# peterWon/D-LIOM

Measured on AMD Instinct MI355X. Metric: scans/sec (64-beam x 1024 pts -> 10 cm 3D submap), higher is better.
Workload: dtype f32 transforms + u16 voxels/u64 sums (rtcsm), f64 (ceres); 1 GPU; config2 W-dense: 64x1024 scan, all returns matched (adaptive voxel filters neutralised), RTCSM3D + CeresScanMatcher3D(hi+lo) + insertion(hi+lo); N_hi=65536, N_lo=65536, C=35937, linear_window=1, angular_window=5, rescored_candidates_last=2, box_kernel_variant=0, map_scans=20, grids_inserted_into=2, parallelism=replicas x1

## Files before the change

d-liom_amd/csrc/internal.h:

```cpp
#ifndef DLIOM_CSRC_INTERNAL_H_
#define DLIOM_CSRC_INTERNAL_H_

#include <hip/hip_runtime.h>

#include <chrono>
#include <cstddef>
#include <cstdint>
#include <memory>
#include <string>
#include <vector>

#include "../../include/dliom.h"
#include "pinned_layout.h"

namespace dliom {

void set_last_error(const char* what, hipError_t e, const char* file, int line);

#define DLIOM_HIP_TRY(expr)                                          \
  do {                                                               \
    hipError_t _e = (expr);                                          \
    if (_e != hipSuccess) {                                          \
      ::dliom::set_last_error(#expr, _e, __FILE__, __LINE__);        \
      return DLIOM_ERR_HIP;                                          \
// ... 89 lines not shown
  int64_t read_backs = 0;
  int64_t poll_fallbacks = 0;
  int64_t host_syncs = 0;
  dliom::DevBuf batch;
  dliom::DevBuf icp_batch;
  dliom::DevBuf ndt_batch;
  dliom::DevBuf ndt_target_batch;
  dliom::DevBuf nn_index_batch;
  dliom::DevBuf xray_leaves, xray_cells;
  dliom::DevBuf surf, surf_out;
  dliom::DevBuf painter;
  int64_t painter_launches = 0, painter_pairs = 0, painter_texels_uploaded = 0;
  dliom::DevBuf compress, compress_out;
  bool surf_tables_ready = false;
  dliom::DevBuf outlier;
  void* batch_pinned = nullptr;
  size_t batch_pinned_bytes = 0;
  int reserve_batch_pinned(size_t bytes);
  int num_cus = 256;
  unsigned func_attr_set = 0;
  hipStream_t aux_stream = nullptr;
  hipEvent_t aux_fork = nullptr;
  dliom::DevBuf aux_scratch;
  void* aux_pinned = nullptr;
  int aux_histogram_size = 0;
  unsigned aux_seq = 0;
  bool aux_enqueued = false;
  const dliom_cloud* aux_cloud = nullptr;
  float aux_rotation[4] = {1.f, 0.f, 0.f, 0.f};
  bool aux_has_rotation = false;
  bool hist_expect_big = true;
  int hist_poll_us = 150;
  std::chrono::steady_clock::time_point hist_enqueued_at;
  hipStream_t hist_big_stream = nullptr;
  hipEvent_t hist_fork = nullptr, hist_join = nullptr;
  bool profiling = false;
  unsigned profiling_mask = ~0u;
  struct Span {
    hipEvent_t a, b;
    int id;
  };
  std::vector<Span> spans;
  std::vector<hipEvent_t> event_pool;
  double kernel_ms[DLIOM_KERNEL_COUNT] = {};
  int64_t kernel_launches[DLIOM_KERNEL_COUNT] = {};
  dliom_rtcsm_stats last_rtcsm = {};
  void* rtcsm_state = nullptr;
  void (*rtcsm_state_free)(void*) = nullptr;

  int begin_span(int id);
  void end_span(int span);
  int collect_spans();
};

struct dliom_grid {
  dliom_ctx* ctx = nullptr;
  float resolution = 0.f;
  int bits = 1;
  uint32_t* d_table = nullptr;
  uint16_t* d_pool = nullptr;
  int32_t* d_slot_coord = nullptr;
  uint32_t* d_count = nullptr;
  int64_t capacity = 0;
  int64_t used_upper = 1;
  unsigned* h_count_slot = nullptr;
  unsigned insert_seq = 0, applied_seq = 0;
// ... 127 lines not shown
int device_block_alloc(int device, size_t need, void** p, size_t* bytes);
void device_block_free(int device, void* p, size_t bytes);
struct CompactScratch {
  unsigned *keep, *inclusive, *max_sq;
  int* index;
  void* tmp;
  size_t tmp_bytes;
  void* extra;
};
int carve_compact(dliom_ctx* ctx, int64_t n, CompactScratch* s, size_t extra_bytes = 0, size_t zeroed_extra_bytes = 0);
int empty_cloud(dliom_ctx* ctx, dliom_cloud** out);
int max_of_kept(dliom_ctx* ctx, const float* x, const float* y, const float* z, int64_t n, const CompactScratch& s);
int scan_kept(dliom_ctx* ctx, int64_t n, const CompactScratch& s);
int read_kept(dliom_ctx* ctx, int64_t n, const CompactScratch& s, const GatherJob* more, int64_t* kept, float* max_sq,
              unsigned* more_host);
int emit_kept(dliom_ctx* ctx, const float* x, const float* y, const float* z, int64_t n, const CompactScratch& s, int64_t kept,
              float max_sq, dliom_cloud** out, int32_t* kept_index);
int compact_kept(dliom_ctx* ctx, const dliom_cloud* in, const CompactScratch& s, const unsigned* flag_word, unsigned* flag,
                 dliom_cloud** out, int32_t* kept_index, int64_t capacity, int64_t* num_kept);
int gather_batch_attributes(dliom_ctx* ctx, const int* d_index, int64_t kept, const float* src_intensities, const float* src_colors,
                            float* dst_intensities, float* dst_colors);
int compact_batch(dliom_points_batch* batch, const CompactScratch& s, const unsigned* flag_word, unsigned* flag, int64_t* num_kept);
struct DevicePoints {
  const float4* xyzt;
  const float* intensities;
};
int assemble_from_sensor_points(dliom_ctx* ctx, dliom_trajectory* traj, int64_t cloud_time, const float* points_xyzt, const DevicePoints* device_points,
                                int64_t n, const double sensor_to_tracking[7], dliom_cloud** out, float origin[3], int32_t* kept_index,
                                int64_t capacity, int64_t* num_kept, const float* intensities, AttrBlock* kept_intensities);
int timed_cloud_view(const dliom_timed_cloud* cloud, const dliom_ctx* ctx, int64_t* n, const float4** d_xyzt, const float** d_intensities,
                     float* front_t);
int timed_cloud_origin_index(const dliom_timed_cloud* cloud, bool* has, const float** d_origin_index);
int std_sort_order_enqueue(dliom_ctx* ctx, const float* d_keys, int n, const int** d_order, const int** d_status);
int launch_sequential_sums(dliom_ctx* ctx, int method, const GridView& gv, const dliom_cloud& cloud, const float4* d_rot,
                           int R, const float* d_trans, const unsigned* d_list, const unsigned* d_count, unsigned count,
                           DevBuf* scratch, float* d_ksums);
int sequential_sum_method(int64_t num_points);
int sequential_probability_sums(dliom_ctx* ctx, const dliom_cloud& cloud, const dliom_grid* grid, const float* poses7,
                                int k, float* sums);
struct SequentialSumJob {
  const dliom_cloud* cloud;
  const dliom_grid* grid;
  int first, k;
};
int sequential_probability_sums_enqueue(dliom_ctx* ctx, const SequentialSumJob* jobs, int num_jobs, const float4* d_rot,
                                        const float* d_trans, const unsigned* d_list, float* d_sums);
}

#endif
```

d-liom_amd/csrc/rtcsm3d.hip:

```cpp
#include <algorithm>
#include <cmath>
#include <cstdio>
#include <cstdlib>
#include <cstring>
#include <type_traits>
#include <vector>

#include <dlfcn.h>
#include <rccl/rccl.h>

#include "device_common.h"
#include "host_math.h"
#include "probability_values.h"
#include "rtcsm_candidates.h"
#include "score_box.h"

namespace dliom {

constexpr int kBlock = 256;

template <int PPT, bool WIDE = false>
__global__ __launch_bounds__(kBlock) void rtcsm_score_kernel(
    GridView g, const float* __restrict__ px, const float* __restrict__ py,
    const float* __restrict__ pz, const float4* __restrict__ rot, int R, int r_first, int r_last,
    const float* __restrict__ trans, int T, int rots_per_block,
    unsigned long long* __restrict__ sums) {
  extern __shared__ unsigned block_sum[];
  float x[PPT], y[PPT], z[PPT];
#pragma unroll
  for (int k = 0; k < PPT; ++k) {
    const int i = (blockIdx.x * PPT + k) * kBlock + threadIdx.x;
    x[k] = px[i];
    y[k] = py[i];
    z[k] = pz[i];
  }
  const int r_begin = r_first + blockIdx.y * rots_per_block;
  const int r_end = min(r_begin + rots_per_block, r_last);
  const int lane = threadIdx.x & 63;
  const float inv = g.inv_resolution;
  typedef typename std::conditional<WIDE, unsigned long long, unsigned>::type idx_t;
  const idx_t sentinel = static_cast<idx_t>(1) << (3 * g.log2_leaves);
  const unsigned lb = static_cast<unsigned>(g.log2_leaves);
  for (int r = r_begin; r < r_end; ++r) {
    for (int j = threadIdx.x; j < T; j += kBlock) block_sum[j] = 0u;
    __syncthreads();
    const float4 qq = rot[r];
// ... 215 lines not shown
              ox[k] = lds_off[min(max(cell_of(rx[k] + t.x, g.resolution) + to_table, 0), TS - 1)];
              oy[k] = lds_off[TS + min(max(cell_of(ry[k] + t.y, g.resolution) + to_table, 0), TS - 1)];
              oz[k] = lds_off[2 * TS + min(max(cell_of(rz[k] + t.z, g.resolution) + to_table, 0), TS - 1)];
            }
          }
        }
        unsigned v[P];
#pragma unroll
        for (int k = 0; k < P; ++k)
          v[k] = *reinterpret_cast<const unsigned short*>(reinterpret_cast<const char*>(g.dense) + (ox[k] + oy[k] + oz[k]));
        unsigned a = 0;
#pragma unroll
        for (int k = 0; k < P; ++k) a += v[k];
        atomicAdd(&lds_acc[jj * bs + threadIdx.x], a);
      }
    }
    if (active) {
      for (int jj = 0; jj < tc; ++jj)
        atomicAdd(&sums[static_cast<size_t>(jc + jj) * R + r],
                  static_cast<unsigned long long>(lds_acc[jj * bs + threadIdx.x]));
    }
  }
}

struct BoundParams {
  double a;
  double b;
  double delta;
  double wt, wr;
  int n;
  int n_pad;
  int R, T;
  int r_first, r_last;
};

__device__ double seq_sum_error_bound(int n, double U) {
  double err = 0.0;
  long long i = 0;
  for (int k = -4; k < 64 && i < n; ++k) {
    const double top = ldexp(1.0, k + 1);
    long long last;
    if (U < top) {
      last = n;
    } else {
      last = static_cast<long long>(floor(top / 0.93)) - 1;
      if (last > n) last = n;
    }
    if (last > i) {
      err += 0.5 * ldexp(1.0, k - 23) * static_cast<double>(last - i);
      i = last;
    }
  }
  return err;
}

__device__ __forceinline__ float next_up(float f) { return __uint_as_float(__float_as_uint(f) + 1u); }
__device__ __forceinline__ float next_down(float f) {
  const unsigned u = __float_as_uint(f);
  return u == 0u ? 0.f : __uint_as_float(u - 1u);
}

__global__ void rtcsm_bounds_kernel(const unsigned long long* __restrict__ sums, long long C,
                                    const float* __restrict__ t_norm, const float* __restrict__ r_angle,
                                    BoundParams p, float* __restrict__ lo, float* __restrict__ hi,
                                    unsigned* __restrict__ best_lo_bits) {
  const long long c = static_cast<long long>(blockIdx.x) * blockDim.x + threadIdx.x;
  const bool in_range = c < C;
  const int j = in_range ? static_cast<int>(c / p.R) : 0, r = in_range ? static_cast<int>(c % p.R) : 0;
  const bool mine = in_range && r >= p.r_first && r < p.r_last;
  float flo = 0.f, fhi = -1.f;
  if (mine) {
  const double s = static_cast<double>(sums[c] - static_cast<unsigned long long>(p.n_pad));
  const double mid = p.a * s + p.b * p.n;
  const double slack = p.delta * p.n + 1e-9 * mid;
  double sum_lo = mid - slack, sum_hi = mid + slack;
  const double U = sum_hi * (1.0 + 1.0 / 32.0);
  const double e = seq_sum_error_bound(p.n, U);
  if (sum_hi + e > U || p.n > (1 << 19)) {
    flo = 0.f;
    fhi = 3.0e38f;
  } else {
    sum_lo -= e;
    sum_hi += e;
    const double arg = static_cast<double>(t_norm[j]) * p.wt + static_cast<double>(r_angle[r]) * p.wr;
    const double pen = exp(-(arg * arg));
    const float nf = static_cast<float>(p.n);
    float qlo = next_down(next_down(static_cast<float>(sum_lo))) / nf;
    float qhi = next_up(next_up(static_cast<float>(sum_hi))) / nf;
    qlo = next_down(qlo);
    qhi = next_up(qhi);
    flo = next_down(next_down(static_cast<float>(static_cast<double>(qlo) * pen * (1.0 - 1e-9))));
    fhi = next_up(next_up(static_cast<float>(static_cast<double>(qhi) * pen * (1.0 + 1e-9))));
    if (!(flo > 0.f)) flo = 0.f;
  }
  }
  if (in_range) {
    lo[c] = flo;
    hi[c] = fhi;
  }
  unsigned best = __float_as_uint(flo);
#pragma unroll
  for (int off = 32; off > 0; off >>= 1) best = max(best, static_cast<unsigned>(__shfl_xor(static_cast<int>(best), off, 64)));
  if ((threadIdx.x & 63) == 0 && best != 0u) atomicMax(best_lo_bits, best);
}

__global__ void rtcsm_select_kernel(const float* __restrict__ hi, long long C,
                                    const unsigned* __restrict__ best_lo_bits,
                                    unsigned* __restrict__ count, unsigned* __restrict__ list) {
  const long long c = static_cast<long long>(blockIdx.x) * blockDim.x + threadIdx.x;
  if (c >= C) return;
// ... 640 lines not shown
                       const dliom_cloud& cloud, const dliom_grid* grid, int shard, int num_shards,
                       unsigned* local_best_lo_bits) {
#ifdef DLIOM_EXPERIMENTS
  g_host_prep.start();
#endif
  if (cloud.n <= 0) return DLIOM_ERR_EMPTY_CLOUD;
  if (cloud.n > (1 << 27) || num_shards < 1 || shard < 0 || shard >= num_shards)
    return DLIOM_ERR_INVALID_ARGUMENT;
  RtcsmState* st = state_of(ctx);
  st->active = false;
  st->o = *o;
  st->cloud = cloud;
  st->grid = grid;
  std::memcpy(st->init7, init7, sizeof st->init7);
  st->shard = shard;
  st->num_shards = num_shards;
  st->used_box = false;
  Candidates& c = st->c;
  generate_candidates(*o, grid->resolution, cloud.max_norm, init7, &c);
  DLIOM_PREP_LAP(0);
  const int64_t C = c.w.num_candidates;
  const int R = static_cast<int>(c.w.num_rotations), T = static_cast<int>(c.w.num_translations);
  if (C <= 0 || C > (int64_t{1} << 31)) return DLIOM_ERR_INVALID_ARGUMENT;
  st->r_first = static_cast<int>(static_cast<int64_t>(R) * shard / num_shards);
  st->r_last = static_cast<int>(static_cast<int64_t>(R) * (shard + 1) / num_shards);

  const size_t bytes_f = align256(static_cast<size_t>(C) * 4);
  DLIOM_TRY(ctx->bounds.reserve(3 * bytes_f + 256));
  char* bb = static_cast<char*>(ctx->bounds.p);
  float* d_lo = reinterpret_cast<float*>(bb);
  st->d_hi = reinterpret_cast<float*>(bb + bytes_f);
  st->d_list = reinterpret_cast<unsigned*>(bb + 2 * bytes_f);
  st->d_ctrs = reinterpret_cast<unsigned*>(bb + 3 * bytes_f);
  const FillJob zero_ctrs{st->d_ctrs, 8, 0u};
  if (st->r_last <= st->r_first) DLIOM_TRY(fill_multi(ctx, &zero_ctrs, 1));
  if (st->r_last > st->r_first) {
    int64_t pad_processed = 0;
    DLIOM_TRY(run_score_volume(ctx, cloud, grid, c, st->r_first, st->r_last, &st->d, &st->d_sums,
                               &pad_processed, &zero_ctrs));
    st->used_box = ctx->last_score_used_box;
    const LutModel& lm = lut_model();
    BoundParams bp;
    bp.a = lm.a;
    bp.b = lm.b;
    bp.delta = lm.delta;
    bp.wt = o->translation_delta_cost_weight;
    bp.wr = o->rotation_delta_cost_weight;
    bp.n = static_cast<int>(cloud.n);
    bp.n_pad = static_cast<int>(pad_processed);
    bp.R = R;
    bp.T = T;
    bp.r_first = st->r_first;
    bp.r_last = st->r_last;
    const unsigned cblocks = static_cast<unsigned>((C + 255) / 256);
    const int span = ctx->begin_span(DLIOM_KERNEL_RTCSM_SELECT);
    hipLaunchKernelGGL(rtcsm_bounds_kernel, dim3(cblocks), dim3(256), 0, ctx->stream, st->d_sums,
                       static_cast<long long>(C), st->d.t_norm, st->d.r_angle, bp, d_lo, st->d_hi,
                       st->d_ctrs);
    ctx->end_span(span);
    DLIOM_HIP_TRY(hipGetLastError());
  }
  if (local_best_lo_bits != nullptr) {
    unsigned* h_err = pinned_at<unsigned>(ctx, kPinBoxErrorWord);
    *h_err = 0u;
    DLIOM_HIP_TRY(hipMemcpyAsync(local_best_lo_bits, st->d_ctrs, 4, hipMemcpyDeviceToHost, ctx->stream));
    if (st->used_box)
      DLIOM_HIP_TRY(hipMemcpyAsync(h_err, static_cast<char*>(ctx->box_error.p) + 4, 4, hipMemcpyDeviceToHost, ctx->stream));
    DLIOM_HIP_TRY(hipStreamSynchronize(ctx->stream));
    bool overflow = false;
    DLIOM_TRY(box_overflowed(ctx, *h_err, &overflow));
    if (overflow && !ctx->force_dense_score) {
      ctx->force_dense_score = true;
      const dliom_rtcsm_options o_copy = st->o;
      const int s = match_begin(ctx, &o_copy, init7, cloud, grid, shard, num_shards, local_best_lo_bits);
      ctx->force_dense_score = false;
      return s;
    }
  }
  st->active = true;
  return DLIOM_OK;
}

static int match_finish(dliom_ctx* ctx, const unsigned* global_best_lo_bits, uint64_t* local_best_packed) {
  RtcsmState* st = state_of(ctx);
  if (!st->active) return DLIOM_ERR_INVALID_ARGUMENT;
  const dliom_rtcsm_options* o = &st->o;
  const Candidates& c = st->c;
  const int64_t C = c.w.num_candidates;
  const int R = static_cast<int>(c.w.num_rotations);
  const dliom_cloud& cloud = st->cloud;
  st->best_score = -1.f;
  st->best_c = -1;
  unsigned K = 0;
  if (st->r_last > st->r_first) {
    if (global_best_lo_bits != nullptr) {
      DLIOM_HIP_TRY(hipMemcpyAsync(st->d_ctrs, global_best_lo_bits, 4, hipMemcpyHostToDevice, ctx->stream));
    }
    const unsigned cblocks = static_cast<unsigned>((C + 255) / 256);
    int span = ctx->begin_span(DLIOM_KERNEL_RTCSM_SELECT);
    hipLaunchKernelGGL(rtcsm_select_kernel, dim3(cblocks), dim3(256), 0, ctx->stream, st->d_hi,
                       static_cast<long long>(C), st->d_ctrs, st->d_ctrs + 1, st->d_list);
    ctx->end_span(span);
    DLIOM_HIP_TRY(hipGetLastError());
  }
  constexpr unsigned kSpecK = 8;
  std::vector<unsigned> list;
  std::vector<float> ksums;
  if (st->r_last > st->r_first) {
    static_assert((2 + 2 * kSpecK + 1) * 4 <= kPinMatchReadback.bytes, "the read-back fits its region");
    unsigned* h_ctrs = pinned_at<unsigned>(ctx, kPinMatchReadback);
    unsigned* h_list = h_ctrs + 2;
    float* h_sums = reinterpret_cast<float*>(h_ctrs + 2 + kSpecK);
    auto rescore = [&](unsigned count, const unsigned* d_count, size_t list_offset) -> int {
      DLIOM_TRY(ctx->rescore.reserve(align256(static_cast<size_t>(count) * 4)));
      const int span = ctx->begin_span(DLIOM_KERNEL_RTCSM_RESCORE);
      const int s = launch_sequential_sums(ctx, sequential_sum_method(cloud.n), st->grid->view(), cloud, st->d.rot, R, st->d.trans,
                                           st->d_list + list_offset, d_count, count, &ctx->misc, ctx->rescore.as<float>());
      ctx->end_span(span);
      return s;
    };
    DLIOM_TRY(rescore(kSpecK, st->d_ctrs + 1, 0));
    unsigned* h_err = h_ctrs + 2 + 2 * kSpecK;
    *h_err = 0u;
    const bool want_err = st->used_box && global_best_lo_bits == nullptr;
    const GatherJob back[4] = {{st->d_ctrs, 2}, {st->d_list, kSpecK}, {ctx->rescore.p, kSpecK},
                               {static_cast<char*>(ctx->box_error.p) + 4, 1}};
    DLIOM_TRY(gather_and_wait(ctx, back, want_err ? 4 : 3, h_ctrs));
    {
      bool overflow = false;
      DLIOM_TRY(box_overflowed(ctx, *h_err, &overflow));
      if (overflow && !ctx->force_dense_score) {
        ctx->force_dense_score = true;
        const dliom_rtcsm_options o_copy = st->o;
        const dliom_cloud cloud_copy = st->cloud;
        double init_copy[7];
        std::memcpy(init_copy, st->init7, sizeof init_copy);
        int s = match_begin(ctx, &o_copy, init_copy, cloud_copy, st->grid, st->shard, st->num_shards, nullptr);
        if (s == DLIOM_OK) s = match_finish(ctx, nullptr, local_best_packed);
        ctx->force_dense_score = false;
        return s;
      }
    }
    K = h_ctrs[1];
    const unsigned first = std::min(K, kSpecK);
    list.assign(h_list, h_list + first);
    ksums.assign(h_sums, h_sums + first);
    if (K > kSpecK) {
      const unsigned rest = K - kSpecK;
      DLIOM_TRY(rescore(rest, nullptr, kSpecK));
      list.resize(K);
      ksums.resize(K);
      DLIOM_HIP_TRY(hipMemcpyAsync(list.data() + kSpecK, st->d_list + kSpecK, static_cast<size_t>(rest) * 4,
                                   hipMemcpyDeviceToHost, ctx->stream));
      DLIOM_HIP_TRY(hipMemcpyAsync(ksums.data() + kSpecK, ctx->rescore.p, static_cast<size_t>(rest) * 4,
                                   hipMemcpyDeviceToHost, ctx->stream));
      DLIOM_HIP_TRY(hipStreamSynchronize(ctx->stream));
    }
  }
  if (K > 0) {
    const int n = static_cast<int>(cloud.n);
    for (unsigned k = 0; k < K; ++k) {
      const int64_t cc = list[k];
      const int j = static_cast<int>(cc / R), r = static_cast<int>(cc % R);
      float score = ksums[k];
      score /= static_cast<float>(n);
      const double arg = c.t_norm[j] * o->translation_delta_cost_weight +
                         c.r_angle[r] * o->rotation_delta_cost_weight;
      score *= std::exp(-(arg * (arg * 1.0)));
      if (score > st->best_score || (score == st->best_score && cc < st->best_c)) {
        st->best_score = score;
        st->best_c = cc;
      }
    }
  }
  ctx->last_rtcsm.window = c.w;
  ctx->last_rtcsm.num_points = cloud.n;
  ctx->last_rtcsm.num_rescored = K;
  ctx->last_rtcsm.score_kernel = ctx->last_score_mapping;
  ctx->last_rtcsm.box_kernel_status = ctx->last_box_refusal;
  ctx->last_rtcsm.box_kernel_variant = ctx->last_box_refusal == DLIOM_BOX_RAN ? ctx->last_box_variant : -1;
  ctx->last_rtcsm.best_index = st->best_c;
  if (local_best_packed != nullptr) {
// ... 340 lines not shown
```

d-liom_amd/csrc/sequential_sums.hip:

```cpp
#include <algorithm>
#include <cstring>
#include <vector>

#include "device_common.h"
#include "probability_values.h"

namespace dliom {

constexpr int kChainTile = 2048;
__global__ __launch_bounds__(256) void rtcsm_rescore_kernel(
    GridView g, const float* __restrict__ px, const float* __restrict__ py,
    const float* __restrict__ pz, int n, const float4* __restrict__ rot, int R,
    const float* __restrict__ trans, const unsigned* __restrict__ list, const unsigned* __restrict__ count,
    float k_scale, float k_offset, float k_unknown, float* __restrict__ sums) {
  __shared__ float4 tile[2][kChainTile / 4];
  if (count != nullptr && blockIdx.x >= *count) return;
  const unsigned c = list[blockIdx.x];
  const int j = static_cast<int>(c / static_cast<unsigned>(R));
  const int r = static_cast<int>(c % static_cast<unsigned>(R));
  const float4 qq = rot[r];
  const Quat4 q{qq.x, qq.y, qq.z, qq.w};
  const float tx = trans[3 * j], ty = trans[3 * j + 1], tz = trans[3 * j + 2];
  const int num_tiles = (n + kChainTile - 1) / kChainTile;
  const int producer = static_cast<int>(threadIdx.x) - 64;
  auto produce = [&](int t) {
    if (producer < 0) return;
    float* dst = reinterpret_cast<float*>(tile[t & 1]);
    for (int k = producer; k < kChainTile; k += 192) {
      const int i = t * kChainTile + k;
      float prob = 0.f;
      if (i < n) {
        float rx, ry, rz;
        rotate_point(q, px[i], py[i], pz[i], rx, ry, rz);
        const unsigned v = grid_value(g, cell_of(rx + tx, g.resolution), cell_of(ry + ty, g.resolution),
                                      cell_of(rz + tz, g.resolution)) & 0x7FFFu;
        prob = v == 0u ? k_unknown : static_cast<float>(static_cast<int>(v)) * k_scale + k_offset;
      }
      dst[k] = prob;
    }
  };
  float s = 0.f;
  produce(0);
  __syncthreads();
  for (int t = 0; t < num_tiles; ++t) {
    if (t + 1 < num_tiles) produce(t + 1);
    if (threadIdx.x == 0) {
      const float4* src = tile[t & 1];
#pragma unroll 8
      for (int k = 0; k < kChainTile / 4; ++k) {
        const float4 v = src[k];
        s += v.x;
        s += v.y;
        s += v.z;
        s += v.w;
      }
    }
    __syncthreads();
  }
  if (threadIdx.x == 0) sums[blockIdx.x] = s;
}

struct ParityFn {
  unsigned s0, s1;
  unsigned p0, p1;
};
__device__ __forceinline__ ParityFn compose(const ParityFn& a, const ParityFn& b) {
  ParityFn r;
  r.s0 = a.s0 + (a.p0 ? b.s1 : b.s0);
  r.p0 = a.p0 ? b.p1 : b.p0;
  r.s1 = a.s1 + (a.p1 ? b.s1 : b.s0);
  r.p1 = a.p1 ? b.p1 : b.p0;
  return r;
}
__device__ __forceinline__ ParityFn shfl_up_fn(const ParityFn& f, int off) {
  ParityFn r;
  r.s0 = __shfl_up(f.s0, off, 64);
  r.s1 = __shfl_up(f.s1, off, 64);
  r.p0 = __shfl_up(f.p0, off, 64);
  r.p1 = __shfl_up(f.p1, off, 64);
  return r;
}

constexpr int kScanThreads = 1024;
constexpr int kSerialPrefix = 256;

__global__ void rtcsm_rescore_values_kernel(GridView g, const float* __restrict__ px,
                                            const float* __restrict__ py, const float* __restrict__ pz,
                                            int n, int n_stride, const float4* __restrict__ rot, int R,
                                            const float* __restrict__ trans, const unsigned* __restrict__ list,
                                            const unsigned* __restrict__ count,
                                            unsigned short* __restrict__ values, float k_scale, float k_offset,
                                            float k_unknown, double* __restrict__ chunk_sums, int num_chunks) {
// ... 217 lines not shown
__device__ __forceinline__ PFn2 pfn2_identity() { return PFn2{0u, 0x80000000u}; }
__device__ __forceinline__ PFn2 pack_fn(const ParityFn& f) { return PFn2{f.s0 | (f.p0 << 31), f.s1 | (f.p1 << 31)}; }
__device__ __forceinline__ PFn2 compose2(const PFn2& x, const PFn2& y) {
  PFn2 r;
  r.a = (x.a & 0x7FFFFFFFu) + (static_cast<int>(x.a) < 0 ? y.b : y.a);
  r.b = (x.b & 0x7FFFFFFFu) + (static_cast<int>(x.b) < 0 ? y.b : y.a);
  return r;
}
template <int kCtrl, int kRowMask>
__device__ __forceinline__ PFn2 dpp_fn(const PFn2& f) {
  PFn2 r;
  r.a = static_cast<unsigned>(__builtin_amdgcn_update_dpp(0, static_cast<int>(f.a), kCtrl, kRowMask, 0xf, false));
  r.b = static_cast<unsigned>(__builtin_amdgcn_update_dpp(static_cast<int>(0x80000000u), static_cast<int>(f.b), kCtrl, kRowMask, 0xf, false));
  return r;
}
__device__ __forceinline__ PFn2 wave_inclusive_scan2(PFn2 f) {
  f = compose2(dpp_fn<0x111, 0xf>(f), f);
  f = compose2(dpp_fn<0x112, 0xf>(f), f);
  f = compose2(dpp_fn<0x114, 0xf>(f), f);
  f = compose2(dpp_fn<0x118, 0xf>(f), f);
  f = compose2(dpp_fn<0x142, 0xa>(f), f);
  f = compose2(dpp_fn<0x143, 0xc>(f), f);
  return f;
}
__device__ __forceinline__ PFn2 wave_shift_right1(const PFn2& f) { return dpp_fn<0x138, 0xf>(f); }
__device__ __forceinline__ PFn2 lane_of(const PFn2& f, int l) {
  return PFn2{static_cast<unsigned>(__builtin_amdgcn_readlane(static_cast<int>(f.a), l)),
              static_cast<unsigned>(__builtin_amdgcn_readlane(static_cast<int>(f.b), l))};
}
__device__ __forceinline__ unsigned apply2(const PFn2& f, unsigned parity) { return (parity ? f.b : f.a) & 0x7FFFFFFFu; }

__global__ __launch_bounds__(kScanThreads) void rtcsm_rescore_chunk_scan_kernel(
    const unsigned short* __restrict__ values, int n, int n_stride, float k_scale, float k_offset, float k_unknown,
    const unsigned* __restrict__ count, const ChunkFns* __restrict__ fns, int num_chunks, float* __restrict__ sums) {
  extern __shared__ unsigned short lds_value[];
  if (count != nullptr && blockIdx.x >= *count) return;
  __shared__ PFn2 wave_total[kScanThreads / 64];
  __shared__ unsigned sh_m, sh_e, sh_i0, sh_cross_t, sh_total, sh_mismatch_t, sh_force_serial;
  constexpr int kEarlyChunks = 128;
  __shared__ ChunkFns early_fns[kEarlyChunks];
  const int tid = threadIdx.x, lane = tid & 63, wave = tid >> 6;
  const ChunkFns none{0xFFFFFFFFu, 0u, 0u, 0u, 0xFFFFFFFFu, 0u, 0u, 0u};
  const ChunkFns cf = tid < num_chunks ? fns[static_cast<size_t>(blockIdx.x) * num_chunks + tid] : none;
  if (tid < kEarlyChunks) early_fns[tid] = cf;
  {
    const uint4* src = reinterpret_cast<const uint4*>(values + static_cast<size_t>(blockIdx.x) * n_stride);
    uint4* dst = reinterpret_cast<uint4*>(lds_value);
    for (int i = tid; i < n_stride / 8; i += kScanThreads) dst[i] = src[i];
  }
  __syncthreads();
  auto prob = [&](unsigned v) { return v == 0u ? k_unknown : static_cast<float>(static_cast<int>(v)) * k_scale + k_offset; };
  auto fixed = [&](unsigned i) { return fixed_of_value(lds_value[i], k_scale, k_offset, k_unknown); };
  const int n0 = min(n, kSerialPrefix);
  if (wave == 0) {
    float s = 0.f;
    if (n0 == kSerialPrefix) {
      float pv[kSerialPrefix / 64];
#pragma unroll
      for (int k = 0; k < kSerialPrefix / 64; ++k) pv[k] = prob(lds_value[k * 64 + lane]);
#pragma unroll
      for (int k = 0; k < kSerialPrefix / 64; ++k)
#pragma unroll
        for (int l = 0; l < 64; ++l) s += __int_as_float(__builtin_amdgcn_readlane(__float_as_int(pv[k]), l));
    } else {
      for (int i = 0; i < n0; ++i) s += prob(lds_value[i]);
    }
    const unsigned b0 = __float_as_uint(s);
    unsigned m = (b0 & 0x7FFFFFu) | 0x800000u, e = (b0 >> 23) - 123u, i0 = static_cast<unsigned>(n0);
    const PFn2 idw = pfn2_identity();
    while (i0 < static_cast<unsigned>(n)) {
      const unsigned c_min = max(13421772u >> e, 1u);
      const unsigned window = min(static_cast<unsigned>(n) - i0, ((1u << 24) - m) / c_min + 2u);
      const unsigned c0 = i0 / kChunk;
      const unsigned i_lim = min(static_cast<unsigned>(n), ((i0 + window + kChunk - 1u) / kChunk) * kChunk);
      const unsigned last_chunk = (i_lim - 1u) / kChunk;
      if (last_chunk - c0 >= 64u || last_chunk >= static_cast<unsigned>(kEarlyChunks)) break;
      const unsigned c = c0 + static_cast<unsigned>(lane);
      const unsigned begin = max(i0, c * kChunk), end = min(i_lim, (c + 1u) * kChunk);
      const bool in_window = begin < end;
      PFn2 f = idw;
      bool mismatch = false;
      if (in_window && lane != 0) {
        const ChunkFns cw = early_fns[c];
        if (cw.e0 == e) f = PFn2{cw.s00 | ((cw.pp0 & 1u) << 31), cw.s01 | ((cw.pp0 >> 1) << 31)};
        else if (cw.e1 == e) f = PFn2{cw.s10 | ((cw.pp1 & 1u) << 31), cw.s11 | ((cw.pp1 >> 1) << 31)};
        else mismatch = true;
      }
      {
        const unsigned he = min(i_lim, (c0 + 1u) * kChunk);
        const unsigned i = i0 + static_cast<unsigned>(lane);
        const PFn2 h = wave_inclusive_scan2(i < he ? pack_fn(element_fn(fixed(i), e)) : idw);
        const PFn2 whole = lane_of(h, 63);
        if (lane == 0) f = whole;
      }
      const PFn2 inc = wave_inclusive_scan2(f);
      const PFn2 excl = wave_shift_right1(inc);
      const unsigned p_start = m & 1u;
      const unsigned mt_start = m + apply2(excl, p_start), mt_end = m + apply2(inc, p_start);
      const unsigned long long cross_mask = __ballot(in_window && mt_end >= (1u << 24) && mt_start < (1u << 24));
      const unsigned long long mism_mask = __ballot(mismatch);
      const int cross_l = cross_mask != 0ull ? __ffsll(static_cast<long long>(cross_mask)) - 1 : 64;
      const int mism_l = mism_mask != 0ull ? __ffsll(static_cast<long long>(mism_mask)) - 1 : 64;
      if (mism_l < cross_l || (cross_l == 64 && mism_l != 64)) break;
      if (cross_l == 64) {
        m = static_cast<unsigned>(__builtin_amdgcn_readlane(static_cast<int>(mt_end), 63));
        i0 = i_lim;
        continue;
      }
      const unsigned cb = static_cast<unsigned>(__builtin_amdgcn_readlane(static_cast<int>(begin), cross_l));
      const unsigned ce = static_cast<unsigned>(__builtin_amdgcn_readlane(static_cast<int>(end), cross_l));
      const unsigned ms = static_cast<unsigned>(__builtin_amdgcn_readlane(static_cast<int>(mt_start), cross_l));
      const unsigned i = cb + static_cast<unsigned>(lane);
      const unsigned a_i = i < ce ? fixed(i) : 0u;
      const PFn2 sc = wave_inclusive_scan2(i < ce ? pack_fn(element_fn(a_i, e)) : idw);
      const PFn2 ex = wave_shift_right1(sc);
      const unsigned ps = ms & 1u;
      const unsigned m_before = ms + apply2(ex, ps), m_after = ms + apply2(sc, ps);
      const unsigned long long crossed = __ballot(i < ce && m_after >= (1u << 24));
      if (crossed == 0ull) break;
      const int first = __ffsll(static_cast<long long>(crossed)) - 1;
      const unsigned mb = static_cast<unsigned>(__builtin_amdgcn_readlane(static_cast<int>(m_before), first));
      const unsigned af = static_cast<unsigned>(__builtin_amdgcn_readlane(static_cast<int>(a_i), first));
      const unsigned long long X = (static_cast<unsigned long long>(mb) << e) + af;
      const unsigned e2 = e + 1u;
      const unsigned long long q2 = X >> e2, f2 = X & ((1ull << e2) - 1ull), h2 = 1ull << e;
      const unsigned long long up = (f2 > h2 || (f2 == h2 && (q2 & 1ull))) ? 1ull : 0ull;
      m = static_cast<unsigned>(q2 + up);
      e = e2;
      i0 = cb + static_cast<unsigned>(first) + 1u;
    }
    if (lane == 0) {
      sh_m = m;
      sh_e = e;
      sh_i0 = i0;
      sh_force_serial = 0u;
    }
  }
  __syncthreads();
  const PFn2 id = pfn2_identity();
// ... 53 lines not shown
      __syncthreads();
      continue;
    }
    if (cross_t == 0xFFFFFFFFu) {
      if (tid == 0) {
        sh_m = m + sh_total;
        sh_i0 = i_lim;
      }
    } else if (static_cast<unsigned>(wave) == (cross_t >> 6)) {
      const int cl = static_cast<int>(cross_t & 63u);
      const unsigned cb = static_cast<unsigned>(__builtin_amdgcn_readlane(static_cast<int>(begin), cl));
      const unsigned ce = static_cast<unsigned>(__builtin_amdgcn_readlane(static_cast<int>(end), cl));
      const unsigned ms = static_cast<unsigned>(__builtin_amdgcn_readlane(static_cast<int>(mt_start), cl));
      const unsigned i = cb + static_cast<unsigned>(lane);
      const PFn2 sc = wave_inclusive_scan2(i < ce ? pack_fn(element_fn(fixed(i), e)) : id);
      const PFn2 ex = wave_shift_right1(sc);
      const unsigned ps = ms & 1u;
      const unsigned m_before = ms + apply2(ex, ps);
      const unsigned m_after = ms + apply2(sc, ps);
      const unsigned long long crossed = __ballot(i < ce && m_after >= (1u << 24));
      const int first = __ffsll(static_cast<long long>(crossed)) - 1;
      if (lane == first) {
        const unsigned long long X = (static_cast<unsigned long long>(m_before) << e) + fixed(i);
        const unsigned e2 = e + 1u;
        const unsigned long long q2 = X >> e2, f2 = X & ((1ull << e2) - 1ull), h2 = 1ull << e;
        const unsigned long long up = (f2 > h2 || (f2 == h2 && (q2 & 1ull))) ? 1ull : 0ull;
        sh_m = static_cast<unsigned>(q2 + up);
        sh_e = e2;
        sh_i0 = i + 1u;
      }
    }
    __syncthreads();
  }
  if (tid == 0) sums[blockIdx.x] = __uint_as_float(((sh_e + 123u) << 23) | (sh_m & 0x7FFFFFu));
}

constexpr int kRescoreMethod = 2;
constexpr int64_t kRescoreSerialMaxPoints = 1024;

int sequential_sum_method(int64_t num_points) { return num_points <= kRescoreSerialMaxPoints ? 0 : kRescoreMethod; }

struct ScratchLayout {
  size_t sums_at, fns_at, bytes;
};
static ScratchLayout scratch_layout(size_t count, int n) {
  const int n_stride = (n + 7) & ~7, num_chunks = (n + kChunk - 1) / kChunk;
  const size_t values_bytes = align256(count * n_stride * 2), sums_bytes = align256(count * num_chunks * 8);
  return {values_bytes, values_bytes + sums_bytes, values_bytes + sums_bytes + count * num_chunks * sizeof(ChunkFns)};
}

int launch_sequential_sums(dliom_ctx* ctx, int method, const GridView& gv, const dliom_cloud& cloud, const float4* d_rot,
                           int R, const float* d_trans, const unsigned* d_list, const unsigned* d_count, unsigned count,
                           DevBuf* scratch, float* d_ksums) {
  const float k_scale = kValueToProbabilityScale, k_offset = kValueToProbabilityOffset, k_unknown = kUnknownProbability;
  const int n = static_cast<int>(cloud.n);
  const int n_stride = (n + 7) & ~7;
  const size_t scan_lds = static_cast<size_t>(n_stride) * 2;
  if (method == 0 || scan_lds > 128 * 1024 || count > 65535) {
    hipLaunchKernelGGL(rtcsm_rescore_kernel, dim3(count), dim3(256), 0, ctx->stream, gv, cloud.d_x, cloud.d_y, cloud.d_z, n,
                       d_rot, R, d_trans, d_list, d_count, k_scale, k_offset, k_unknown, d_ksums);
    DLIOM_HIP_TRY(hipGetLastError());
    return DLIOM_OK;
  }
  const int num_chunks = (n + kChunk - 1) / kChunk;
  const ScratchLayout at = scratch_layout(count, n);
  DLIOM_TRY(scratch->reserve(at.bytes));
  char* base = static_cast<char*>(scratch->p);
  unsigned short* d_values = reinterpret_cast<unsigned short*>(base);
  double* d_chunk_sums = method == 2 ? reinterpret_cast<double*>(base + at.sums_at) : nullptr;
  ChunkFns* d_fns = reinterpret_cast<ChunkFns*>(base + at.fns_at);
  hipLaunchKernelGGL(rtcsm_rescore_values_kernel, dim3((n_stride + 255) / 256, count), dim3(256), 0, ctx->stream, gv,
                     cloud.d_x, cloud.d_y, cloud.d_z, n, n_stride, d_rot, R, d_trans, d_list, d_count, d_values, k_scale,
                     k_offset, k_unknown, d_chunk_sums, num_chunks);
  if (method == 2) {
    hipLaunchKernelGGL(rtcsm_rescore_chunk_fns_kernel, dim3((num_chunks + 3) / 4, count), dim3(256), 0, ctx->stream, d_values,
                       n, n_stride, k_scale, k_offset, k_unknown, d_count, d_chunk_sums, num_chunks, d_fns);
    hipLaunchKernelGGL(rtcsm_rescore_chunk_scan_kernel, dim3(count), dim3(kScanThreads), scan_lds, ctx->stream, d_values, n,
                       n_stride, k_scale, k_offset, k_unknown, d_count, d_fns, num_chunks, d_ksums);
  } else {
    hipLaunchKernelGGL(rtcsm_rescore_scan_kernel, dim3(count), dim3(kScanThreads), scan_lds, ctx->stream, d_values, n, n_stride,
                       k_scale, k_offset, k_unknown, d_count, d_ksums);
  }
  DLIOM_HIP_TRY(hipGetLastError());
  return DLIOM_OK;
}

int sequential_probability_sums(dliom_ctx* ctx, const dliom_cloud& cloud, const dliom_grid* grid, const float* poses7,
                                int k, float* sums) {
  if (k <= 0 || k > 65535 || cloud.n <= 0) return DLIOM_ERR_INVALID_ARGUMENT;
  const size_t K = static_cast<size_t>(k);
  const size_t rot_bytes = align256(K * 16), trans_bytes = align256(K * 12), list_bytes = align256(K * 4);
  DLIOM_TRY(ctx->bounds.reserve(rot_bytes + trans_bytes + list_bytes));
  std::vector<char> host(rot_bytes + trans_bytes + list_bytes, 0);
  float* hr = reinterpret_cast<float*>(host.data());
  float* ht = reinterpret_cast<float*>(host.data() + rot_bytes);
  unsigned* hl = reinterpret_cast<unsigned*>(host.data() + rot_bytes + trans_bytes);
  for (size_t i = 0; i < K; ++i) {
    const float* p = poses7 + 7 * i;
    hr[4 * i] = p[3];
    hr[4 * i + 1] = p[4];
    hr[4 * i + 2] = p[5];
    hr[4 * i + 3] = p[6];
    ht[3 * i] = p[0];
    ht[3 * i + 1] = p[1];
    ht[3 * i + 2] = p[2];
    hl[i] = static_cast<unsigned>(i * K + i);
  }
  char* base = static_cast<char*>(ctx->bounds.p);
  DLIOM_HIP_TRY(hipMemcpyAsync(base, host.data(), host.size(), hipMemcpyHostToDevice, ctx->stream));
  const float4* d_rot = reinterpret_cast<const float4*>(base);
  const float* d_trans = reinterpret_cast<const float*>(base + rot_bytes);
// ... 37 lines not shown
```

Before: 973.5 scans/s.

## Publish rescore results from kernel via done-word and precompute error bound table

The rescore kernels now write the candidate list, sums, counters and the error word straight into pinned host memory. The last-arriving block then sets a done word, so the host polls that word with an adaptive interval instead of issuing a gather copy and a stream sync. The per-thread sequential-sum error bound loop in the bounds kernel is replaced by a host-filled table indexed by the exponent of U. The chunk scan kernel stops staging values into LDS, reads from global memory instead, and adds 64-chunk super-function skipping. Risks include correctness of the system-scope fences in the cross-block arrival counter and extra global loads in the scan.

```diff
diff --git a/d-liom_amd/csrc/internal.h b/d-liom_amd/csrc/internal.h
--- a/d-liom_amd/csrc/internal.h
+++ b/d-liom_amd/csrc/internal.h
@@ -145,6 +145,7 @@
   bool hist_expect_big = true;
   int hist_poll_us = 150;
   std::chrono::steady_clock::time_point hist_enqueued_at;
+  int match_poll_us = 150;
   hipStream_t hist_big_stream = nullptr;
   hipEvent_t hist_fork = nullptr, hist_join = nullptr;
   bool profiling = false;
@@ -338,9 +339,18 @@
                      float* front_t);
 int timed_cloud_origin_index(const dliom_timed_cloud* cloud, bool* has, const float** d_origin_index);
 int std_sort_order_enqueue(dliom_ctx* ctx, const float* d_keys, int n, const int** d_order, const int** d_status);
+struct SumReadback {
+  unsigned* dst = nullptr;
+  const unsigned* ctrs = nullptr;
+  const unsigned* err_word = nullptr;
+  unsigned* arrivals = nullptr;
+  unsigned* done_word = nullptr;
+  unsigned done_seq = 0;
+  unsigned slots = 0;
+};
 int launch_sequential_sums(dliom_ctx* ctx, int method, const GridView& gv, const dliom_cloud& cloud, const float4* d_rot,
                            int R, const float* d_trans, const unsigned* d_list, const unsigned* d_count, unsigned count,
-                           DevBuf* scratch, float* d_ksums);
+                           DevBuf* scratch, float* d_ksums, const SumReadback* readback = nullptr);
 int sequential_sum_method(int64_t num_points);
 int sequential_probability_sums(dliom_ctx* ctx, const dliom_cloud& cloud, const dliom_grid* grid, const float* poses7,
                                 int k, float* sums);
diff --git a/d-liom_amd/csrc/rtcsm3d.hip b/d-liom_amd/csrc/rtcsm3d.hip
--- a/d-liom_amd/csrc/rtcsm3d.hip
+++ b/d-liom_amd/csrc/rtcsm3d.hip
@@ -1,4 +1,5 @@
 #include <algorithm>
+#include <chrono>
 #include <cmath>
 #include <cstdio>
 #include <cstdlib>
@@ -12,6 +13,7 @@
 #include "device_common.h"
 #include "host_math.h"
 #include "probability_values.h"
+#include "rtcsm_bounds.h"
 #include "rtcsm_candidates.h"
 #include "score_box.h"
 
@@ -293,27 +295,8 @@
   int n_pad;
   int R, T;
   int r_first, r_last;
+  SeqSumBoundTable err;
 };
-
-__device__ double seq_sum_error_bound(int n, double U) {
-  double err = 0.0;
-  long long i = 0;
-  for (int k = -4; k < 64 && i < n; ++k) {
-    const double top = ldexp(1.0, k + 1);
-    long long last;
-    if (U < top) {
-      last = n;
-    } else {
-      last = static_cast<long long>(floor(top / 0.93)) - 1;
-      if (last > n) last = n;
-    }
-    if (last > i) {
-      err += 0.5 * ldexp(1.0, k - 23) * static_cast<double>(last - i);
-      i = last;
-    }
-  }
-  return err;
-}
 
 __device__ __forceinline__ float next_up(float f) { return __uint_as_float(__float_as_uint(f) + 1u); }
 __device__ __forceinline__ float next_down(float f) {
@@ -336,7 +319,7 @@
   const double slack = p.delta * p.n + 1e-9 * mid;
   double sum_lo = mid - slack, sum_hi = mid + slack;
   const double U = sum_hi * (1.0 + 1.0 / 32.0);
-  const double e = seq_sum_error_bound(p.n, U);
+  const double e = p.err.err[seq_sum_bound_index(U)];
   if (sum_hi + e > U || p.n > (1 << 19)) {
     flo = 0.f;
     fhi = 3.0e38f;
@@ -1043,7 +1026,7 @@
   st->d_hi = reinterpret_cast<float*>(bb + bytes_f);
   st->d_list = reinterpret_cast<unsigned*>(bb + 2 * bytes_f);
   st->d_ctrs = reinterpret_cast<unsigned*>(bb + 3 * bytes_f);
-  const FillJob zero_ctrs{st->d_ctrs, 8, 0u};
+  const FillJob zero_ctrs{st->d_ctrs, 12, 0u};
   if (st->r_last <= st->r_first) DLIOM_TRY(fill_multi(ctx, &zero_ctrs, 1));
   if (st->r_last > st->r_first) {
     int64_t pad_processed = 0;
@@ -1063,6 +1046,7 @@
     bp.T = T;
     bp.r_first = st->r_first;
     bp.r_last = st->r_last;
+    fill_seq_sum_bound_table(bp.n, &bp.err);
     const unsigned cblocks = static_cast<unsigned>((C + 255) / 256);
     const int span = ctx->begin_span(DLIOM_KERNEL_RTCSM_SELECT);
     hipLaunchKernelGGL(rtcsm_bounds_kernel, dim3(cblocks), dim3(256), 0, ctx->stream, st->d_sums,
@@ -1122,21 +1106,38 @@
     unsigned* h_ctrs = pinned_at<unsigned>(ctx, kPinMatchReadback);
     unsigned* h_list = h_ctrs + 2;
     float* h_sums = reinterpret_cast<float*>(h_ctrs + 2 + kSpecK);
-    auto rescore = [&](unsigned count, const unsigned* d_count, size_t list_offset) -> int {
+    auto rescore = [&](unsigned count, const unsigned* d_count, size_t list_offset, const SumReadback* readback) -> int {
       DLIOM_TRY(ctx->rescore.reserve(align256(static_cast<size_t>(count) * 4)));
       const int span = ctx->begin_span(DLIOM_KERNEL_RTCSM_RESCORE);
       const int s = launch_sequential_sums(ctx, sequential_sum_method(cloud.n), st->grid->view(), cloud, st->d.rot, R, st->d.trans,
-                                           st->d_list + list_offset, d_count, count, &ctx->misc, ctx->rescore.as<float>());
+                                           st->d_list + list_offset, d_count, count, &ctx->misc, ctx->rescore.as<float>(), readback);
       ctx->end_span(span);
       return s;
     };
-    DLIOM_TRY(rescore(kSpecK, st->d_ctrs + 1, 0));
     unsigned* h_err = h_ctrs + 2 + 2 * kSpecK;
     *h_err = 0u;
     const bool want_err = st->used_box && global_best_lo_bits == nullptr;
-    const GatherJob back[4] = {{st->d_ctrs, 2}, {st->d_list, kSpecK}, {ctx->rescore.p, kSpecK},
-                               {static_cast<char*>(ctx->box_error.p) + 4, 1}};
-    DLIOM_TRY(gather_and_wait(ctx, back, want_err ? 4 : 3, h_ctrs));
+    if (ctx->done_word != nullptr) {
+      SumReadback rb;
+      rb.dst = h_ctrs;
+      rb.ctrs = st->d_ctrs;
+      rb.err_word = want_err ? reinterpret_cast<const unsigned*>(static_cast<char*>(ctx->box_error.p) + 4) : nullptr;
+      rb.arrivals = st->d_ctrs + 2;
+      rb.done_word = ctx->done_word;
+      rb.done_seq = next_done_seq(ctx);
+      rb.slots = kSpecK;
+      DLIOM_TRY(rescore(kSpecK, st->d_ctrs + 1, 0, &rb));
+      const auto t0 = std::chrono::steady_clock::now();
+      const int s = wait_done(ctx, ctx->stream, ctx->done_word, rb.done_seq, ctx->match_poll_us);
+      const double took_us = std::chrono::duration<double, std::micro>(std::chrono::steady_clock::now() - t0).count();
+      ctx->match_poll_us = static_cast<int>(std::min(4000.0, std::max(150.0, 2.0 * took_us)));
+      DLIOM_TRY(s);
+    } else {
+      DLIOM_TRY(rescore(kSpecK, st->d_ctrs + 1, 0, nullptr));
+      const GatherJob back[4] = {{st->d_ctrs, 2}, {st->d_list, kSpecK}, {ctx->rescore.p, kSpecK},
+                                 {static_cast<char*>(ctx->box_error.p) + 4, 1}};
+      DLIOM_TRY(gather_and_wait(ctx, back, want_err ? 4 : 3, h_ctrs));
+    }
     {
       bool overflow = false;
       DLIOM_TRY(box_overflowed(ctx, *h_err, &overflow));
@@ -1158,7 +1159,7 @@
     ksums.assign(h_sums, h_sums + first);
     if (K > kSpecK) {
       const unsigned rest = K - kSpecK;
-      DLIOM_TRY(rescore(rest, nullptr, kSpecK));
+      DLIOM_TRY(rescore(rest, nullptr, kSpecK, nullptr));
       list.resize(K);
       ksums.resize(K);
       DLIOM_HIP_TRY(hipMemcpyAsync(list.data() + kSpecK, st->d_list + kSpecK, static_cast<size_t>(rest) * 4,
diff --git a/d-liom_amd/csrc/rtcsm_bounds.h b/d-liom_amd/csrc/rtcsm_bounds.h
--- /dev/null
+++ b/d-liom_amd/csrc/rtcsm_bounds.h
@@ -0,0 +1,55 @@
+#ifndef DLIOM_CSRC_RTCSM_BOUNDS_H_
+#define DLIOM_CSRC_RTCSM_BOUNDS_H_
+
+#include <cmath>
+#include <cstdint>
+#include <cstring>
+
+#if defined(__HIPCC__)
+#define DLIOM_BOUNDS_HD __host__ __device__
+#else
+#define DLIOM_BOUNDS_HD
+#endif
+
+namespace dliom {
+
+DLIOM_BOUNDS_HD inline double seq_sum_error_bound(int n, double U) {
+  double err = 0.0;
+  long long i = 0;
+  for (int k = -4; k < 64 && i < n; ++k) {
+    const double top = ldexp(1.0, k + 1);
+    long long last;
+    if (U < top) {
+      last = n;
+    } else {
+      last = static_cast<long long>(floor(top / 0.93)) - 1;
+      if (last > n) last = n;
+    }
+    if (last > i) {
+      err += 0.5 * ldexp(1.0, k - 23) * static_cast<double>(last - i);
+      i = last;
+    }
+  }
+  return err;
+}
+
+constexpr int kSeqSumBoundFirstBinade = -4;
+constexpr int kSeqSumBoundBinades = 68;
+struct SeqSumBoundTable {
+  double err[kSeqSumBoundBinades];
+};
+inline void fill_seq_sum_bound_table(int n, SeqSumBoundTable* t) {
+  for (int K = 0; K < kSeqSumBoundBinades; ++K) t->err[K] = seq_sum_error_bound(n, ldexp(1.0, K + kSeqSumBoundFirstBinade));
+}
+DLIOM_BOUNDS_HD inline int seq_sum_bound_index(double U) {
+  if (!(U > 0.0)) return U == U ? 0 : kSeqSumBoundBinades - 1;
+  uint64_t bits;
+  memcpy(&bits, &U, 8);
+  const int K = static_cast<int>((bits >> 52) & 0x7ffu) - 1023;
+  const int idx = K - kSeqSumBoundFirstBinade;
+  return idx < 0 ? 0 : (idx >= kSeqSumBoundBinades ? kSeqSumBoundBinades - 1 : idx);
+}
+
+}
+
+#endif
diff --git a/d-liom_amd/csrc/sequential_sums.hip b/d-liom_amd/csrc/sequential_sums.hip
--- a/d-liom_amd/csrc/sequential_sums.hip
+++ b/d-liom_amd/csrc/sequential_sums.hip
@@ -6,15 +6,36 @@
 #include "probability_values.h"
 
 namespace dliom {
+
+__device__ __forceinline__ void publish_sum(const SumReadback& rb, const unsigned* __restrict__ list, bool has_sum, float sum) {
+  if (rb.dst == nullptr) return;
+  const unsigned k = blockIdx.x;
+  if (has_sum && k < rb.slots) {
+    rb.dst[2u + k] = list[k];
+    rb.dst[2u + rb.slots + k] = __float_as_uint(sum);
+  }
+  __threadfence_system();
+  if (atomicAdd(rb.arrivals, 1u) == gridDim.x - 1u) {
+    *rb.arrivals = 0u;
+    rb.dst[0] = rb.ctrs[0];
+    rb.dst[1] = rb.ctrs[1];
+    if (rb.err_word != nullptr) rb.dst[2u + 2u * rb.slots] = *rb.err_word;
+    __threadfence_system();
+    *reinterpret_cast<volatile unsigned*>(rb.done_word) = rb.done_seq;
+  }
+}
 
 constexpr int kChainTile = 2048;
 __global__ __launch_bounds__(256) void rtcsm_rescore_kernel(
     GridView g, const float* __restrict__ px, const float* __restrict__ py,
     const float* __restrict__ pz, int n, const float4* __restrict__ rot, int R,
     const float* __restrict__ trans, const unsigned* __restrict__ list, const unsigned* __restrict__ count,
-    float k_scale, float k_offset, float k_unknown, float* __restrict__ sums) {
+    float k_scale, float k_offset, float k_unknown, float* __restrict__ sums, SumReadback rb) {
   __shared__ float4 tile[2][kChainTile / 4];
-  if (count != nullptr && blockIdx.x >= *count) return;
+  if (count != nullptr && blockIdx.x >= *count) {
+    if (threadIdx.x == 0) publish_sum(rb, list, false, 0.f);
+    return;
+  }
   const unsigned c = list[blockIdx.x];
   const int j = static_cast<int>(c / static_cast<unsigned>(R));
   const int r = static_cast<int>(c % static_cast<unsigned>(R));
@@ -57,7 +78,10 @@
     }
     __syncthreads();
   }
-  if (threadIdx.x == 0) sums[blockIdx.x] = s;
+  if (threadIdx.x == 0) {
+    sums[blockIdx.x] = s;
+    publish_sum(rb, list, true, s);
+  }
 }
 
 struct ParityFn {
@@ -341,38 +365,55 @@
 
 __global__ __launch_bounds__(kScanThreads) void rtcsm_rescore_chunk_scan_kernel(
     const unsigned short* __restrict__ values, int n, int n_stride, float k_scale, float k_offset, float k_unknown,
-    const unsigned* __restrict__ count, const ChunkFns* __restrict__ fns, int num_chunks, float* __restrict__ sums) {
-  extern __shared__ unsigned short lds_value[];
-  if (count != nullptr && blockIdx.x >= *count) return;
+    const unsigned* __restrict__ count, const ChunkFns* __restrict__ fns, int num_chunks, float* __restrict__ sums,
+    const unsigned* __restrict__ list, SumReadback rb) {
+  if (count != nullptr && blockIdx.x >= *count) {
+    if (threadIdx.x == 0) publish_sum(rb, list, false, 0.f);
+    return;
+  }
   __shared__ PFn2 wave_total[kScanThreads / 64];
   __shared__ unsigned sh_m, sh_e, sh_i0, sh_cross_t, sh_total, sh_mismatch_t, sh_force_serial;
-  constexpr int kEarlyChunks = 128;
-  __shared__ ChunkFns early_fns[kEarlyChunks];
+  __shared__ uint4 lds_fn[kScanThreads];
+  __shared__ unsigned lds_fn_e[kScanThreads];
+  __shared__ unsigned super_e[kScanThreads / 64][2];
+  __shared__ PFn2 super_fn[kScanThreads / 64][2];
   const int tid = threadIdx.x, lane = tid & 63, wave = tid >> 6;
   const ChunkFns none{0xFFFFFFFFu, 0u, 0u, 0u, 0xFFFFFFFFu, 0u, 0u, 0u};
   const ChunkFns cf = tid < num_chunks ? fns[static_cast<size_t>(blockIdx.x) * num_chunks + tid] : none;
-  if (tid < kEarlyChunks) early_fns[tid] = cf;
+  const unsigned short* __restrict__ vals = values + static_cast<size_t>(blockIdx.x) * n_stride;
   {
-    const uint4* src = reinterpret_cast<const uint4*>(values + static_cast<size_t>(blockIdx.x) * n_stride);
-    uint4* dst = reinterpret_cast<uint4*>(lds_value);
-    for (int i = tid; i < n_stride / 8; i += kScanThreads) dst[i] = src[i];
+    const PFn2 cf0{cf.s00 | ((cf.pp0 & 1u) << 31), cf.s01 | ((cf.pp0 >> 1) << 31)};
+    const PFn2 cf1{cf.s10 | ((cf.pp1 & 1u) << 31), cf.s11 | ((cf.pp1 >> 1) << 31)};
+    lds_fn[tid] = make_uint4(cf0.a, cf0.b, cf1.a, cf1.b);
+    lds_fn_e[tid] = (cf.e0 & 0xFFu) | ((cf.e1 & 0xFFu) << 8);
+#pragma unroll
+    for (int k = 0; k < 2; ++k) {
+      const unsigned E = static_cast<unsigned>(__builtin_amdgcn_readlane(static_cast<int>(k == 0 ? cf.e0 : cf.e1), 0));
+      const bool has0 = cf.e0 == E, has = E != 0xFFFFFFFFu && (has0 || cf.e1 == E);
+      const PFn2 total = lane_of(wave_inclusive_scan2(has ? (has0 ? cf0 : cf1) : pfn2_identity()), 63);
+      const bool all = __ballot(has) == ~0ull;
+      if (lane == 0) {
+        super_e[wave][k] = all ? E : 0xFFFFFFFFu;
+        super_fn[wave][k] = total;
+      }
+    }
   }
   __syncthreads();
   auto prob = [&](unsigned v) { return v == 0u ? k_unknown : static_cast<float>(static_cast<int>(v)) * k_scale + k_offset; };
-  auto fixed = [&](unsigned i) { return fixed_of_value(lds_value[i], k_scale, k_offset, k_unknown); };
+  auto fixed = [&](unsigned i) { return fixed_of_value(vals[i], k_scale, k_offset, k_unknown); };
   const int n0 = min(n, kSerialPrefix);
   if (wave == 0) {
     float s = 0.f;
     if (n0 == kSerialPrefix) {
       float pv[kSerialPrefix / 64];
 #pragma unroll
-      for (int k = 0; k < kSerialPrefix / 64; ++k) pv[k] = prob(lds_value[k * 64 + lane]);
+      for (int k = 0; k < kSerialPrefix / 64; ++k) pv[k] = prob(vals[k * 64 + lane]);
 #pragma unroll
       for (int k = 0; k < kSerialPrefix / 64; ++k)
 #pragma unroll
         for (int l = 0; l < 64; ++l) s += __int_as_float(__builtin_amdgcn_readlane(__float_as_int(pv[k]), l));
     } else {
-      for (int i = 0; i < n0; ++i) s += prob(lds_value[i]);
+      for (int i = 0; i < n0; ++i) s += prob(vals[i]);
     }
     const unsigned b0 = __float_as_uint(s);
     unsigned m = (b0 & 0x7FFFFFu) | 0x800000u, e = (b0 >> 23) - 123u, i0 = static_cast<unsigned>(n0);
@@ -383,19 +424,21 @@
       const unsigned c0 = i0 / kChunk;
       const unsigned i_lim = min(static_cast<unsigned>(n), ((i0 + window + kChunk - 1u) / kChunk) * kChunk);
       const unsigned last_chunk = (i_lim - 1u) / kChunk;
-      if (last_chunk - c0 >= 64u || last_chunk >= static_cast<unsigned>(kEarlyChunks)) break;
+      const unsigned cend = last_chunk - c0 < 64u ? last_chunk + 1u : ((c0 >> 6) + 1u) << 6;
       const unsigned c = c0 + static_cast<unsigned>(lane);
       const unsigned begin = max(i0, c * kChunk), end = min(i_lim, (c + 1u) * kChunk);
-      const bool in_window = begin < end;
+      const bool in_window = c < cend;
+      const bool resume_partial = (i0 & (kChunk - 1u)) != 0u;
       PFn2 f = idw;
       bool mismatch = false;
-      if (in_window && lane != 0) {
-        const ChunkFns cw = early_fns[c];
-        if (cw.e0 == e) f = PFn2{cw.s00 | ((cw.pp0 & 1u) << 31), cw.s01 | ((cw.pp0 >> 1) << 31)};
-        else if (cw.e1 == e) f = PFn2{cw.s10 | ((cw.pp1 & 1u) << 31), cw.s11 | ((cw.pp1 >> 1) << 31)};
+      if (in_window && !(resume_partial && lane == 0)) {
+        const unsigned ce = lds_fn_e[c];
+        const uint4 cw = lds_fn[c];
+        if ((ce & 0xFFu) == e) f = PFn2{cw.x, cw.y};
+        else if ((ce >> 8) == e) f = PFn2{cw.z, cw.w};
         else mismatch = true;
       }
-      {
+      if (resume_partial) {
         const unsigned he = min(i_lim, (c0 + 1u) * kChunk);
         const unsigned i = i0 + static_cast<unsigned>(lane);
         const PFn2 h = wave_inclusive_scan2(i < he ? pack_fn(element_fn(fixed(i), e)) : idw);
@@ -413,7 +456,31 @@
       if (mism_l < cross_l || (cross_l == 64 && mism_l != 64)) break;
       if (cross_l == 64) {
         m = static_cast<unsigned>(__builtin_amdgcn_readlane(static_cast<int>(mt_end), 63));
-        i0 = i_lim;
+        i0 = min(i_lim, cend * kChunk);
+        if (i0 >= i_lim) continue;
+        const unsigned s_first = cend >> 6, s_last = last_chunk >> 6;
+        const bool whole_last = (last_chunk & 63u) == 63u;
+        const unsigned sc = static_cast<unsigned>(lane);
+        const bool active = sc >= s_first && sc <= s_last;
+        PFn2 g = idw;
+        bool stop = active;
+        if (active && (sc < s_last || whole_last)) {
+          if (super_e[sc][0] == e) {
+            g = super_fn[sc][0];
+            stop = false;
+          } else if (super_e[sc][1] == e) {
+            g = super_fn[sc][1];
+            stop = false;
+          }
+        }
+        const PFn2 ginc = wave_inclusive_scan2(g);
+        const PFn2 gexc = wave_shift_right1(ginc);
+        const unsigned gp = m & 1u;
+        const unsigned g_start = m + apply2(gexc, gp), g_end = m + apply2(ginc, gp);
+        const unsigned long long halt_mask = __ballot(active && (stop || g_end >= (1u << 24)));
+        const int halt = halt_mask != 0ull ? __ffsll(static_cast<long long>(halt_mask)) - 1 : static_cast<int>(s_last) + 1;
+        m = static_cast<unsigned>(__builtin_amdgcn_readlane(static_cast<int>(g_start), halt));
+        i0 = min(i_lim, static_cast<unsigned>(halt) * (64u * kChunk));
         continue;
       }
       const unsigned cb = static_cast<unsigned>(__builtin_amdgcn_readlane(static_cast<int>(begin), cross_l));
@@ -533,7 +600,11 @@
     }
     __syncthreads();
   }
-  if (tid == 0) sums[blockIdx.x] = __uint_as_float(((sh_e + 123u) << 23) | (sh_m & 0x7FFFFFu));
+  if (tid == 0) {
+    const float sum = __uint_as_float(((sh_e + 123u) << 23) | (sh_m & 0x7FFFFFu));
+    sums[blockIdx.x] = sum;
+    publish_sum(rb, list, true, sum);
+  }
 }
 
 constexpr int kRescoreMethod = 2;
@@ -552,14 +623,15 @@
 
 int launch_sequential_sums(dliom_ctx* ctx, int method, const GridView& gv, const dliom_cloud& cloud, const float4* d_rot,
                            int R, const float* d_trans, const unsigned* d_list, const unsigned* d_count, unsigned count,
-                           DevBuf* scratch, float* d_ksums) {
+                           DevBuf* scratch, float* d_ksums, const SumReadback* readback) {
+  const SumReadback rb = readback != nullptr ? *readback : SumReadback{};
   const float k_scale = kValueToProbabilityScale, k_offset = kValueToProbabilityOffset, k_unknown = kUnknownProbability;
   const int n = static_cast<int>(cloud.n);
   const int n_stride = (n + 7) & ~7;
   const size_t scan_lds = static_cast<size_t>(n_stride) * 2;
   if (method == 0 || scan_lds > 128 * 1024 || count > 65535) {
     hipLaunchKernelGGL(rtcsm_rescore_kernel, dim3(count), dim3(256), 0, ctx->stream, gv, cloud.d_x, cloud.d_y, cloud.d_z, n,
-                       d_rot, R, d_trans, d_list, d_count, k_scale, k_offset, k_unknown, d_ksums);
+                       d_rot, R, d_trans, d_list, d_count, k_scale, k_offset, k_unknown, d_ksums, rb);
     DLIOM_HIP_TRY(hipGetLastError());
     return DLIOM_OK;
   }
@@ -576,8 +648,8 @@
   if (method == 2) {
     hipLaunchKernelGGL(rtcsm_rescore_chunk_fns_kernel, dim3((num_chunks + 3) / 4, count), dim3(256), 0, ctx->stream, d_values,
                        n, n_stride, k_scale, k_offset, k_unknown, d_count, d_chunk_sums, num_chunks, d_fns);
-    hipLaunchKernelGGL(rtcsm_rescore_chunk_scan_kernel, dim3(count), dim3(kScanThreads), scan_lds, ctx->stream, d_values, n,
-                       n_stride, k_scale, k_offset, k_unknown, d_count, d_fns, num_chunks, d_ksums);
+    hipLaunchKernelGGL(rtcsm_rescore_chunk_scan_kernel, dim3(count), dim3(kScanThreads), 0, ctx->stream, d_values, n,
+                       n_stride, k_scale, k_offset, k_unknown, d_count, d_fns, num_chunks, d_ksums, d_list, rb);
   } else {
     hipLaunchKernelGGL(rtcsm_rescore_scan_kernel, dim3(count), dim3(kScanThreads), scan_lds, ctx->stream, d_values, n, n_stride,
                        k_scale, k_offset, k_unknown, d_count, d_ksums);
```

After: 1036 scans/s, median of 6. +6.4%, better.
